# probably-nothing-labs/denormalized

Measured on AMD Instinct MI355X. Metric: rows/sec through window()+filter() on synthetic sensor stream, higher is better.
Workload: dtype f64

## Files before the change

### denormalized_amd/csrc/dz_internal.h

```cpp
#pragma once
#include <cstddef>
#include <cstdint>
#include <type_traits>
#include <hip/hip_runtime.h>

namespace dz {

constexpr int NB = 512;
constexpr int LOG_NB = 9;
constexpr int BLOCK = 256;
constexpr int WAVES_PER_BLOCK = BLOCK / 64;
constexpr int MAX_RANGES = 4096;
constexpr int ST_RECORDS = 2048;
constexpr int INTERN_STAGE_BYTES = 4096;

constexpr uint32_t META_KLOC_MASK = 0xFFFFu;
constexpr int META_WIDX_SHIFT = 16;
constexpr uint32_t META_WIDX_MASK = 0xFFFu;
constexpr int META_VALID_SHIFT = 28;

struct WinParams {
    int64_t s0;
    int64_t len_ms;
    int64_t slide_ms;
    int32_t nw;
    int32_t is_sliding;
};

struct FoldChunk {
    int32_t w_lo, w_hi;
    int32_t k_lo, k_hi;
    int64_t kcap;
    uint64_t row_base;
    int32_t bin_stride;
    int32_t tl_nw;
};

constexpr int MAX_EXTRA_COLS = 3;
struct FoldExtras {
    const double* vals[MAX_EXTRA_COLS] = {};
    const uint8_t* valid[MAX_EXTRA_COLS] = {};
    uint64_t* slab = nullptr;
    int64_t cells = 0;
    int32_t nx = 0;
};

void launch_gen(hipStream_t stream, uint64_t seed, int64_t t0, int64_t start_row,
                int64_t n, int64_t nkeys, int64_t rows_per_ms,
                int64_t* d_ts, int64_t* d_keys, int32_t* d_kid, double* d_vals);

void launch_intern(hipStream_t stream, const int32_t* d_offs, const char* d_data,
                   int64_t n,
                   uint4* tab ,
                   uint32_t* tab_row, uint32_t p_mask, uint32_t* id_off,
                   uint32_t* id_len, char* pool,
                   uint32_t* ctrs ,
                   uint32_t id_cap, uint32_t pool_cap, int32_t* out_kid,
                   uint32_t seq ,
                   uint64_t fp_mask ,
                   uint32_t* d_dbg);

void launch_intern_i64(hipStream_t stream, const int64_t* d_keys, int64_t n,
                       uint4* tab ,
                       uint32_t p_mask, int64_t* ikeys ,
                       uint32_t* ctrs ,
                       uint32_t id_cap, int32_t* out_kid,
                       uint32_t seq ,
                       uint64_t fp_mask ,
                       uint32_t* d_dbg);

void launch_gen_utf8(hipStream_t stream, uint64_t seed, int64_t start_row,
                     int64_t n, int64_t nkeys, int32_t* d_lens,
                     const int32_t* d_offs, char* d_data);

void launch_minmax(hipStream_t stream, const int64_t* d_ts, const int32_t* d_kid,
                   int64_t n, uint64_t* d_scalars);

void launch_hist(hipStream_t stream, const int32_t* d_kid, const int64_t* d_ts,
                 int64_t n, int64_t chunk, int C, const WinParams& wp,
                 uint32_t* d_ghist, uint64_t* d_scalars );

constexpr int SCAN_SSPLIT = 32;
void launch_scan(hipStream_t stream, const uint32_t* d_ghist, int C,
                 uint32_t* d_psum, uint32_t* d_bucket_base ,
                 uint32_t* d_gofs);

void launch_scatter(hipStream_t stream, const int32_t* d_kid, const int64_t* d_ts,
                    const double* d_vals, const uint8_t* d_validity ,
                    int64_t n, int64_t chunk, int C, int32_t st_rows,
                    const WinParams& wp, const uint32_t* d_gofs, uint4* d_grec,
                    uint32_t rec_limit, uint32_t* d_dbg );

constexpr int FOLD_GCAP = 256;

void launch_regroup_fold(hipStream_t stream, const uint4* d_grec,
                         const uint32_t* d_bucket_base,
                         const FoldChunk& fc, const int32_t* d_slot_of_widx,
                         uint64_t* s_cnt, double* s_min, double* s_max,
                         double* s_sum, uint64_t* s_first, int64_t slab_cells,
                         uint32_t* d_dbg, double* v_base, int64_t vslab_cells,
                         const FoldExtras& fx);

void launch_regroup_l1(hipStream_t stream, const uint4* d_grec,
                       const uint32_t* d_bucket_base,
                       const FoldChunk& fc, uint32_t* d_b1offs,
                       uint32_t* d_b1lens, uint4* d_grec2);

void launch_regroup_l2_fold(hipStream_t stream, const uint4* d_grec2,
                            const uint32_t* d_bucket_base,
                            const FoldChunk& fc, int nb1,
                            const uint32_t* d_b1offs, const uint32_t* d_b1lens,
                            const int32_t* d_slot_of_widx, uint64_t* s_cnt,
                            double* s_min, double* s_max, double* s_sum,
                            uint64_t* s_first, int64_t slab_cells,
                            uint32_t* d_dbg, double* v_base,
                            int64_t vslab_cells, const FoldExtras& fx);

struct EGatherSlots {
    int32_t s[16];
    uint64_t base[16];
};

struct EmitFilter {
    int32_t on;
    int32_t field;
    int32_t cmp;
    double lit;
};

__host__ __device__ inline bool emit_filter_pass(const EmitFilter& ef,
                                                 uint64_t cnt, double mn,
                                                 double mx, double sum) {
    double v;
// ... 50 lines not shown

void launch_emission_slabread(hipStream_t stream, const uint64_t* slab_first,
                              const uint64_t* slab_cnt, const double* slab_min,
                              const double* slab_max, const double* slab_sum,
                              uint64_t base, int64_t K, uint64_t* ekeys, uint32_t* ekid,
                              uint64_t* fkeys, uint32_t* fkid, uint32_t* fiota,
                              uint32_t* counter, uint32_t* counter2,
                              const EmitFilter& ef, uint64_t* ocnt, double* omin,
                              double* omax, double* osum, double* oavg,
                              uint8_t* oflags);
void launch_emission_sort(hipStream_t stream, int64_t K, uint64_t* fkeys,
                          uint64_t* skeys, uint32_t* fiota, uint32_t* okid,
                          uint32_t* counter2, uint32_t* rhist, uint32_t* roffs,
                          uint64_t max_key );
void launch_emission_group_read(hipStream_t stream, const uint64_t* s_base,
                                int64_t stride_u64, const EGatherSlots& slots,
                                int gcount, int64_t K, int64_t kcap,
                                const EmitFilter& ef, int cshift,
                                uint64_t* gkeys, uint32_t* gkid,
                                uint32_t* giota, uint64_t* gcnt_col,
                                double* gmin, double* gmax, double* gsum,
                                double* gavg, uint8_t* gflags, uint32_t* gtot,
                                uint32_t* gcnt);
void launch_emission_group_sort(hipStream_t stream, int64_t elem_cap,
                                int gcount, int cshift, uint64_t max_first,
                                uint64_t* gkeys, uint64_t* gskeys,
                                uint32_t* gkid, uint32_t* gokid,
                                uint32_t* giota, uint64_t* gcnt_col,
                                double* gmin, double* gmax, double* gsum,
                                double* gavg, uint8_t* gflags, uint32_t* gtot,
                                uint32_t* rhist, uint32_t* roffs, char* pout);

void launch_esort_small(hipStream_t stream, uint64_t* fkeys, uint64_t* skeys,
                        uint32_t* fiota, uint32_t* okid, uint32_t* counter2,
                        uint64_t max_key);
constexpr int EMIT_RCHUNK = 4096;
constexpr int EMIT_RBINS = 2048;

void launch_reset_slots(hipStream_t stream, const int32_t* d_slots, int ns,
                        int64_t kcap, uint64_t* s_cnt, uint64_t* s_first);

void launch_reset_slots_x(hipStream_t stream, const int32_t* d_slots, int ns,
                          int nx, int64_t kcap, uint64_t* x_slab);

void launch_egather_slabs(hipStream_t stream, const uint64_t* s_base,
                          int64_t stride_u64, EGatherSlots slots, int gcount,
                          uint64_t* out);
void launch_egather_slabs_var(hipStream_t stream, const uint64_t* s_base,
                              const double* v_base, int64_t kcap,
                              EGatherSlots slots, int gcount, uint64_t* out);
void launch_egather_slabs_x(hipStream_t stream, const uint64_t* s_base,
                            const uint64_t* x_slab, int nx, int64_t kcap,
                            EGatherSlots slots, int gcount, uint64_t* out);
void launch_arm_scalars(hipStream_t stream, uint64_t* scalars);

void launch_fill_i64(hipStream_t stream, int64_t* d_p, int64_t n, int64_t v);

struct JsonFields {
    char ts_name[32];
    char key_name[32];
    char val_name[32];
    int32_t ts_len, key_len, val_len;
};
void launch_json_count(hipStream_t stream, const char* d_buf, int64_t nbytes,
                       int C, int64_t chunk, int32_t tail_record,
                       uint32_t* d_cnt, uint32_t* d_base, uint32_t* d_tot);
void launch_json_parse(hipStream_t stream, const char* d_buf, int64_t nbytes,
                       int C, int64_t chunk, const JsonFields& jf,
                       const uint32_t* d_base, const uint32_t* d_tot,
                       int64_t* d_recoff, int64_t nrec, int64_t* o_ts,
                       int64_t* o_kbeg, int32_t* o_klen, double* o_val,
                       uint32_t* d_blocksum, uint32_t* d_ktot, int32_t* o_koff,
                       char* o_kdata, uint32_t* d_dbg);
void launch_gen_json(hipStream_t stream, uint64_t seed, int64_t t0,
                     int64_t start_row, int64_t n, int64_t nkeys,
                     int64_t rows_per_ms, int32_t* d_lens,
                     const int64_t* d_offs, char* d_data);

void launch_join_precheck(hipStream_t stream, const int64_t* d_trips,
                          const int64_t* d_drivers, int64_t n,
                          const int64_t* tab_trip, uint64_t p_mask,
                          uint32_t* d_pre);
void launch_join_build(hipStream_t stream, const int64_t* d_trips,
                       const int64_t* d_drivers, int64_t n, int64_t* tab_trip,
                       int64_t* tab_drv, uint64_t p_mask, uint32_t* d_dbg,
                       uint32_t* d_pre);
void launch_join_probe(hipStream_t stream, const int64_t* d_ts,
                       const int64_t* d_trips, const double* d_vals, int64_t n,
                       int64_t chunk, int C, const int64_t* tab_trip,
                       const int64_t* tab_drv, uint64_t p_mask,
                       int32_t* d_drvtmp, uint32_t* d_jcnt, uint32_t* d_mbase,
                       uint32_t* d_ubase, uint32_t* d_tot, int64_t* o_ts,
                       int32_t* o_kid, double* o_val, int64_t ubuf_base,
                       int64_t* u_ts, int64_t* u_trip, double* u_val);
void launch_zero_counters(hipStream_t stream, uint32_t* two_u32);
void launch_emission_permute(hipStream_t stream, int64_t K,
                             const uint32_t* counter2, const uint32_t* sidx,
                             const uint32_t* fkid, const uint64_t* ocnt,
                             const double* omin, const double* omax,
                             const double* osum, const double* oavg,
                             const uint8_t* oflags, char* out);

}
```

### denormalized_amd/csrc/kernels.hip

```cpp
#include "dz_internal.h"

#include <algorithm>

namespace dz {

__device__ __forceinline__ int64_t i64min(int64_t a, int64_t b) { return a < b ? a : b; }


__device__ __forceinline__ uint64_t splitmix64(uint64_t x) {
    x += 0x9e3779b97f4a7c15ULL;
    x = (x ^ (x >> 30)) * 0xbf58476d1ce4e5b9ULL;
    x = (x ^ (x >> 27)) * 0x94d049bb133111ebULL;
    return x ^ (x >> 31);
}

__device__ __forceinline__ int64_t snap_ms(int64_t ts, int64_t len_ms) {
    int64_t len_s = len_ms / 1000;
    if (len_s == 0) return ts - (ts % len_ms);
    return (ts / 1000) / len_s * len_s * 1000;
}

__device__ __forceinline__ int64_t floordiv(int64_t a, int64_t b) {
    int64_t q = a / b, r = a % b;
    return q - ((r != 0) & ((r < 0) != (b < 0)));
// ... 37 lines not shown
    if (blocks < 1) blocks = 1;
    hipLaunchKernelGGL(k_gen, dim3(blocks), dim3(BLOCK), 0, s, seed, t0,
                       start_row, n, nkeys, rows_per_ms, d_ts, d_keys, d_kid, d_vals);
}


__device__ __forceinline__ uint64_t fnv1a64(const char* p, int32_t len) {
    uint64_t h = 1469598103934665603ULL;
    for (int32_t i = 0; i < len; i++) {
        h ^= (uint8_t)p[i];
        h *= 1099511628211ULL;
    }
    return h;
}

__device__ __forceinline__ bool bytes_eq(const char* a, const char* b,
                                         int32_t len) {
    for (int32_t i = 0; i < len; i++)
        if (a[i] != b[i]) return false;
    return true;
}

constexpr uint32_t INTERN_INLINE_MAX = 16;

__device__ __forceinline__ uint64_t slot_fp(const uint4& v) {
    return (uint64_t)v.x | ((uint64_t)v.y << 32);
}

__device__ __forceinline__ uint64_t key_fp_bytes(const uint8_t* p, int32_t len,
                                                 uint64_t* klo, uint64_t* khi) {
    uint64_t lo = 0, hi = 0, fp = 1469598103934665603ULL;
    if ((uint32_t)len <= INTERN_INLINE_MAX) {
        const int32_t n0 = len < 8 ? len : 8;
        for (int32_t j = 0; j < n0; j++) {
            const uint64_t b = p[j];
            fp = (fp ^ b) * 1099511628211ULL;
            lo |= b << (8 * j);
        }
        for (int32_t j = 8; j < len; j++) {
            const uint64_t b = p[j];
            fp = (fp ^ b) * 1099511628211ULL;
            hi |= b << (8 * (j - 8));
        }
    } else {
        fp = fnv1a64((const char*)p, len);
    }
    *klo = lo;
    *khi = hi;
    return fp;
}

constexpr int INTERN_STAGE_GRAN = INTERN_STAGE_BYTES / 16 + 2;

__global__ __launch_bounds__(BLOCK) void k_intern_claim(const int32_t* offs,
        const char* data, int64_t n, uint4* tab, uint32_t* tab_row,
        const uint32_t* id_off, const uint32_t* id_len,
        const char* pool, uint32_t p_mask, uint64_t fp_mask, int32_t* out_kid,
        uint32_t* fresh_seq, uint32_t seq, uint32_t* dbg) {
    __shared__ int32_t s_offs[BLOCK + 1];
    __shared__ uint4 s_stage[INTERN_STAGE_GRAN];
    const int t = threadIdx.x;
    const int64_t ntiles = (n + BLOCK - 1) / BLOCK;
    for (int64_t tile = blockIdx.x; tile < ntiles; tile += gridDim.x) {
        const int64_t i0 = tile * BLOCK;
        const int rows = (int)i64min(BLOCK, n - i0);
        if (t < rows) s_offs[t] = offs[i0 + t];
        if (t == 0) s_offs[rows] = offs[i0 + rows];
        __syncthreads();
        const int32_t o_first = s_offs[0];
        const uint32_t span = (uint32_t)(s_offs[rows] - o_first);
        const bool staged = span <= (uint32_t)INTERN_STAGE_BYTES;
        uint32_t head = 0;
        if (staged) {
            if (span) {
                const char* a0 = data + o_first;
                head = (uint32_t)((uintptr_t)a0 & 15u);
                const uint4* g = (const uint4*)(a0 - head);
                const uint32_t ngran = (head + span + 15u) >> 4;
                for (uint32_t k = t; k < ngran; k += BLOCK) s_stage[k] = g[k];
            }
            __syncthreads();
        }
        const bool active = t < rows;
        const int64_t i = i0 + t;
        int32_t o0 = 0, len = 0;
        uint64_t klo = 0, khi = 0, fp = 0;
        if (active) {
            o0 = s_offs[t];
            len = s_offs[t + 1] - o0;
            if (staged) {
                const uint32_t q = head + (uint32_t)(o0 - o_first);
                fp = key_fp_bytes((const uint8_t*)s_stage + q, len, &klo,
                                  &khi);
            } else {
                fp = key_fp_bytes((const uint8_t*)data + o0, len, &klo, &khi);
            }
        }
        __syncthreads();
        if (!active) continue;
        const char* p = data + o0;
        fp &= fp_mask;
        if (!fp) fp = 1;
        uint32_t slot = (uint32_t)fp & p_mask;
        int32_t out;
        for (uint32_t probes = 0;; slot = (slot + 1) & p_mask) {
            const uint4 a = tab[(size_t)slot * 2];
            const uint4 b = tab[(size_t)slot * 2 + 1];
            const uint32_t cand = a.z;
            const uint32_t lo = a.w;
            const bool assigned = cand != ~0u;
            const bool fpeq = slot_fp(a) == fp;
            const uint64_t slo = (uint64_t)b.x | ((uint64_t)b.y << 32);
            const uint64_t shi = (uint64_t)b.z | ((uint64_t)b.w << 32);
            const bool inline_hit = assigned & fpeq &
                ((uint32_t)len <= INTERN_INLINE_MAX) &
                (lo == (((uint32_t)len << 6) | 63u)) & (slo == klo) &
                (shi == khi);
            if (inline_hit) {
                out = (int32_t)cand;
                break;
            }
            if (assigned) {
                const uint32_t clen = lo & 63u;
                const bool is_inline =
                    clen == 63u && (lo >> 6) <= INTERN_INLINE_MAX;
                if (fpeq && !is_inline) {
                    const bool fits = clen != 63u;
                    const uint32_t co = fits ? (lo >> 6) : id_off[cand];
                    const uint32_t cl = fits ? clen : id_len[cand];
                    if (cl == (uint32_t)len && bytes_eq(pool + co, p, len)) {
                        out = (int32_t)cand;
                        break;
                    }
                }
            } else {
                uint64_t got = __hip_atomic_load(
                    (const uint64_t*)tab + (size_t)slot * 4, __ATOMIC_RELAXED,
                    __HIP_MEMORY_SCOPE_AGENT);
                if (got == 0)
                    got = (uint64_t)atomicCAS(
                        (unsigned long long*)&tab[(size_t)slot * 2], 0ULL,
                        (unsigned long long)fp);
                if (got == 0 || got == fp) {
                    if (got == 0) tab_row[slot] = (uint32_t)i;
                    *fresh_seq = seq;
                    out = ~(int32_t)slot;
                    break;
                }
            }
            if (++probes > p_mask) {
                dbg[3] = 4;
                *fresh_seq = seq;
                out = ~(int32_t)slot;
                break;
            }
        }
        out_kid[i] = out;
    }
}

__global__ __launch_bounds__(BLOCK) void k_intern_assign(uint4* tab,
        uint32_t* tab_row, uint32_t p_count,
        const int32_t* offs, const char* data, uint32_t* id_off,
        uint32_t* id_len, char* pool, uint32_t* ctrs, uint32_t id_cap,
        uint32_t pool_cap, const uint32_t* fresh_seq, uint32_t seq,
        uint32_t* dbg) {
    if (*fresh_seq != seq) return;
    int64_t stride = (int64_t)gridDim.x * blockDim.x;
    for (int64_t sl = blockIdx.x * (int64_t)blockDim.x + threadIdx.x;
         sl < p_count; sl += stride) {
        uint4 v = tab[(size_t)sl * 2];
        if (slot_fp(v) == 0 || v.z != ~0u) continue;
        const uint32_t r = tab_row[sl];
        const int32_t o0 = offs[r];
        const int32_t len = offs[r + 1] - o0;
        const uint32_t nid = atomicAdd(&ctrs[0], 1u);
        const uint32_t po = atomicAdd(&ctrs[1], (uint32_t)len);
        if (nid >= id_cap || po + (uint32_t)len > pool_cap) {
            dbg[3] = nid >= id_cap ? 1 : 2;
            continue;
        }
        uint64_t klo = 0, khi = 0;
        for (int32_t j = 0; j < len; j++) {
            const uint8_t c = (uint8_t)data[o0 + j];
            pool[po + j] = (char)c;
            if (j < 8) klo |= (uint64_t)c << (8 * j);
            else if (j < (int32_t)INTERN_INLINE_MAX)
                khi |= (uint64_t)c << (8 * (j - 8));
        }
        id_off[nid] = po;
        id_len[nid] = (uint32_t)len;
        v.z = nid;
        if ((uint32_t)len <= INTERN_INLINE_MAX) {
            v.w = ((uint32_t)len << 6) | 63u;
            tab[(size_t)sl * 2 + 1] = make_uint4((uint32_t)klo,
                (uint32_t)(klo >> 32), (uint32_t)khi, (uint32_t)(khi >> 32));
        } else {
            v.w = (len <= 62 && po < (1u << 26)) ? ((po << 6) | (uint32_t)len)
                                                 : 0xFFFFFFFFu;
        }
        tab[(size_t)sl * 2] = v;
    }
}

__global__ __launch_bounds__(BLOCK) void k_intern_lookup(const int32_t* offs,
        const char* data, int64_t n, const uint4* tab,
        const uint32_t* id_off, const uint32_t* id_len, const char* pool,
        int32_t* out_kid, const uint32_t* fresh_seq, uint32_t seq,
        uint32_t* dbg) {
    if (*fresh_seq != seq) return;
    int64_t stride = (int64_t)gridDim.x * blockDim.x;
    for (int64_t i = blockIdx.x * (int64_t)blockDim.x + threadIdx.x; i < n;
         i += stride) {
        const int32_t v = out_kid[i];
        if (v >= 0) continue;
        const uint32_t slot = (uint32_t)~v;
        const uint32_t cand = tab[(size_t)slot * 2].z;
        int32_t id = 0;
        if (cand == ~0u) {
            dbg[3] = 5;
        } else {
            const int32_t o0 = offs[i];
            const int32_t len = offs[i + 1] - o0;
            const bool eq = id_len[cand] == (uint32_t)len &&
                            bytes_eq(pool + id_off[cand], data + o0, len);
            if (eq) id = (int32_t)cand;
            else dbg[3] = 6;
        }
        out_kid[i] = id;
    }
}

void launch_intern(hipStream_t s, const int32_t* d_offs, const char* d_data,
                   int64_t n, uint4* tab, uint32_t* tab_row, uint32_t p_mask,
                   uint32_t* id_off, uint32_t* id_len, char* pool,
                   uint32_t* ctrs, uint32_t id_cap, uint32_t pool_cap,
                   int32_t* out_kid, uint32_t seq, uint64_t fp_mask,
                   uint32_t* dbg) {
    int blocks = (int)std::min<int64_t>((n + BLOCK - 1) / BLOCK, 2048);
    if (blocks < 1) blocks = 1;
    const uint32_t P = p_mask + 1;
    int sblocks = (int)std::min<uint32_t>((P + BLOCK - 1) / BLOCK, 2048);
    uint32_t* fresh_seq = ctrs + 2;
    hipLaunchKernelGGL(k_intern_claim, dim3(blocks), dim3(BLOCK), 0, s, d_offs,
                       d_data, n, tab, tab_row, id_off, id_len,
                       pool, p_mask, fp_mask, out_kid, fresh_seq, seq, dbg);
    hipLaunchKernelGGL(k_intern_assign, dim3(sblocks), dim3(BLOCK), 0, s,
                       tab, tab_row, P, d_offs, d_data, id_off,
                       id_len, pool, ctrs, id_cap, pool_cap, fresh_seq, seq,
                       dbg);
    hipLaunchKernelGGL(k_intern_lookup, dim3(blocks), dim3(BLOCK), 0, s,
                       d_offs, d_data, n, tab, id_off,
                       id_len, pool, out_kid, fresh_seq, seq, dbg);
}


constexpr uint64_t I64_ZERO_CLAIM = 1;

__global__ __launch_bounds__(BLOCK) void k_intern_i64_claim(
        const int64_t* keys, int64_t n, uint4* tab, uint32_t p_mask,
        uint64_t fp_mask, int32_t* out_kid, uint32_t* fresh_seq, uint32_t seq,
        uint32_t* dbg) {
    const int64_t stride = (int64_t)gridDim.x * blockDim.x;
    for (int64_t i = blockIdx.x * (int64_t)blockDim.x + threadIdx.x; i < n;
         i += stride) {
        const uint64_t key = (uint64_t)keys[i];
        const bool zero = key == 0;
        const uint64_t want = zero ? I64_ZERO_CLAIM : key;
        uint32_t slot = zero ? p_mask + 1
                             : (uint32_t)(splitmix64(key) & fp_mask) & p_mask;
        int32_t out;
        for (uint32_t probes = 0;; slot = (slot + 1) & p_mask) {
            const uint4 a = tab[slot];
            if (a.z != ~0u) {
                if (slot_fp(a) == want) {
                    out = (int32_t)a.z;
                    break;
                }
            } else {
                uint64_t got = __hip_atomic_load(
                    (const uint64_t*)tab + (size_t)slot * 2, __ATOMIC_RELAXED,
                    __HIP_MEMORY_SCOPE_AGENT);
                if (got == 0)
                    got = (uint64_t)atomicCAS((unsigned long long*)&tab[slot],
                                              0ULL, (unsigned long long)want);
                if (got == 0 || got == want) {
                    if (got == 0) ((uint32_t*)&tab[slot])[3] = (uint32_t)i;
                    *fresh_seq = seq;
                    out = ~(int32_t)slot;
                    break;
                }
            }
            if (++probes > p_mask) {
                dbg[3] = 4;
                *fresh_seq = seq;
                out = ~(int32_t)slot;
                break;
            }
        }
// ... 56 lines not shown
                       n, tab, out_kid, fresh_seq, seq, dbg);
}

__device__ __forceinline__ int32_t dec_digits(uint64_t k) {
    int32_t d = 1;
    while (k >= 10) { k /= 10; d++; }
    return d;
}

__global__ void k_gen_keylens(uint64_t seed, int64_t start_row, int64_t n,
                              int64_t nkeys, int32_t* lens) {
    int64_t stride = (int64_t)gridDim.x * blockDim.x;
    for (int64_t i = blockIdx.x * (int64_t)blockDim.x + threadIdx.x; i < n;
         i += stride) {
        uint64_t r = splitmix64(seed ^ (0x9e3779b97f4a7c15ULL *
                                        (uint64_t)(start_row + i + 1)));
        lens[i] = 7 + dec_digits(r % (uint64_t)nkeys);
    }
}

__global__ void k_gen_keyfill(uint64_t seed, int64_t start_row, int64_t n,
                              int64_t nkeys, const int32_t* offs, char* data) {
    const char* pfx = "sensor_";
    int64_t stride = (int64_t)gridDim.x * blockDim.x;
    for (int64_t i = blockIdx.x * (int64_t)blockDim.x + threadIdx.x; i < n;
         i += stride) {
        uint64_t r = splitmix64(seed ^ (0x9e3779b97f4a7c15ULL *
                                        (uint64_t)(start_row + i + 1)));
        uint64_t k = r % (uint64_t)nkeys;
        char* p = data + offs[i];
        for (int j = 0; j < 7; j++) p[j] = pfx[j];
        int32_t len = offs[i + 1] - offs[i];
        for (int32_t j = len - 1; j >= 7; j--) {
            p[j] = (char)('0' + (k % 10));
            k /= 10;
        }
    }
}

void launch_gen_utf8(hipStream_t s, uint64_t seed, int64_t start_row, int64_t n,
                     int64_t nkeys, int32_t* d_lens, const int32_t* d_offs,
                     char* d_data) {
    int blocks = (int)std::min<int64_t>((n + BLOCK - 1) / BLOCK, 2048);
    if (blocks < 1) blocks = 1;
    if (d_lens)
        hipLaunchKernelGGL(k_gen_keylens, dim3(blocks), dim3(BLOCK), 0, s, seed,
                           start_row, n, nkeys, d_lens);
    if (d_data)
        hipLaunchKernelGGL(k_gen_keyfill, dim3(blocks), dim3(BLOCK), 0, s, seed,
                           start_row, n, nkeys, d_offs, d_data);
}


__device__ __forceinline__ uint64_t map_i64(int64_t x) {
    return (uint64_t)x ^ 0x8000000000000000ULL;
}

__global__ __launch_bounds__(BLOCK) void k_minmax(const int64_t* ts,
        const int32_t* kid, int64_t n, uint64_t* scalars) {
    __shared__ uint64_t red[3][WAVES_PER_BLOCK];
    uint64_t mn = ~0ULL, mx = 0, km = 0;
    int64_t stride = (int64_t)gridDim.x * blockDim.x;
    for (int64_t i = blockIdx.x * (int64_t)blockDim.x + threadIdx.x; i < n; i += stride) {
        uint64_t t = map_i64(ts[i]);
        mn = min(mn, t);
        mx = max(mx, t);
        if (kid) km = max(km, (uint64_t)(uint32_t)kid[i]);
    }
    for (int o = 32; o > 0; o >>= 1) {
        mn = min(mn, (uint64_t)__shfl_down((unsigned long long)mn, o));
        mx = max(mx, (uint64_t)__shfl_down((unsigned long long)mx, o));
        km = max(km, (uint64_t)__shfl_down((unsigned long long)km, o));
    }
    const int wave = threadIdx.x >> 6;
    if ((threadIdx.x & 63) == 0) {
        red[0][wave] = mn;
        red[1][wave] = mx;
        red[2][wave] = km;
    }
    __syncthreads();
    if (threadIdx.x == 0) {
        for (int w = 1; w < WAVES_PER_BLOCK; w++) {
            mn = min(mn, red[0][w]);
            mx = max(mx, red[1][w]);
            km = max(km, red[2][w]);
        }
        atomicMin((unsigned long long*)&scalars[0], (unsigned long long)mn);
        atomicMax((unsigned long long*)&scalars[1], (unsigned long long)mx);
        atomicMax((unsigned long long*)&scalars[2], (unsigned long long)km);
    }
}

void launch_minmax(hipStream_t s, const int64_t* d_ts, const int32_t* d_kid,
                   int64_t n, uint64_t* d_scalars) {
    int blocks = (int)std::min<int64_t>((n + BLOCK - 1) / BLOCK, 512);
    if (blocks < 1) blocks = 1;
    hipLaunchKernelGGL(k_minmax, dim3(blocks), dim3(BLOCK), 0, s, d_ts, d_kid, n,
                       d_scalars);
}


__global__ __launch_bounds__(BLOCK) void k_hist(const int32_t* kid,
        const int64_t* ts, int64_t n, int64_t chunk, WinParams wp,
        uint32_t* ghist, uint64_t* scalars) {
    __shared__ uint32_t h[NB];
    __shared__ uint64_t red[3][WAVES_PER_BLOCK];
    for (int t = threadIdx.x; t < NB; t += BLOCK) h[t] = 0;
    __syncthreads();
    int64_t lo = blockIdx.x * chunk;
    int64_t hi = i64min(n, lo + chunk);
    uint64_t mn = ~0ULL, mx = 0, km = 0;
    for (int64_t i = lo + threadIdx.x; i < hi; i += BLOCK) {
        uint32_t k = (uint32_t)kid[i];
        uint32_t m = 1;
        if (wp.is_sliding) {
            int32_t jm, mm;
            row_windows(ts[i], wp, &jm, &mm);
            m = (uint32_t)mm;
        }
        if (scalars) {
            uint64_t t = map_i64(ts[i]);
            mn = min(mn, t);
            mx = max(mx, t);
            km = max(km, (uint64_t)k);
        }
        if (m) atomicAdd(&h[k & (NB - 1)], m);
    }
    __syncthreads();
    for (int t = threadIdx.x; t < NB; t += BLOCK)
        ghist[(int64_t)blockIdx.x * NB + t] = h[t];
    if (scalars) {
        for (int o = 32; o > 0; o >>= 1) {
            mn = min(mn, (uint64_t)__shfl_down((unsigned long long)mn, o));
            mx = max(mx, (uint64_t)__shfl_down((unsigned long long)mx, o));
            km = max(km, (uint64_t)__shfl_down((unsigned long long)km, o));
        }
        const int wave = threadIdx.x >> 6;
        if ((threadIdx.x & 63) == 0) {
            red[0][wave] = mn;
            red[1][wave] = mx;
            red[2][wave] = km;
        }
        __syncthreads();
        if (threadIdx.x == 0) {
            for (int w = 1; w < WAVES_PER_BLOCK; w++) {
                mn = min(mn, red[0][w]);
                mx = max(mx, red[1][w]);
                km = max(km, red[2][w]);
            }
            atomicMin((unsigned long long*)&scalars[0], (unsigned long long)mn);
            atomicMax((unsigned long long*)&scalars[1], (unsigned long long)mx);
            atomicMax((unsigned long long*)&scalars[2], (unsigned long long)km);
        }
    }
}

void launch_hist(hipStream_t s, const int32_t* d_kid, const int64_t* d_ts,
                 int64_t n, int64_t chunk, int C, const WinParams& wp,
                 uint32_t* d_ghist, uint64_t* d_scalars) {
    hipLaunchKernelGGL(k_hist, dim3(C), dim3(BLOCK), 0, s, d_kid, d_ts, n, chunk,
                       wp, d_ghist, d_scalars);
}


constexpr int SSPLIT = SCAN_SSPLIT;

__global__ void k_scan_partial(const uint32_t* ghist, int C, int cs,
                               uint32_t* psum) {
    int bkt = blockIdx.x * blockDim.x + threadIdx.x;
    int seg = blockIdx.y;
    if (bkt >= NB) return;
    int c0 = seg * cs, c1 = min(C, c0 + cs);
    uint32_t s = 0;
    for (int c = c0; c < c1; c++) s += ghist[(int64_t)c * NB + bkt];
    psum[(int64_t)seg * NB + bkt] = s;
}

__global__ __launch_bounds__(NB) void k_scan_base(const uint32_t* psum,
                                                  uint32_t* base) {
    __shared__ uint32_t part[NB];
    const int bkt = threadIdx.x;
    uint32_t t = 0;
    for (int g = 0; g < SSPLIT; g++) t += psum[(int64_t)g * NB + bkt];
    part[bkt] = t;
    __syncthreads();
    for (int o = 1; o < NB; o <<= 1) {
        uint32_t v = (bkt >= o) ? part[bkt - o] : 0;
        __syncthreads();
        part[bkt] += v;
        __syncthreads();
    }
    base[bkt] = bkt ? part[bkt - 1] : 0;
    if (bkt == NB - 1) base[NB] = part[NB - 1];
}

__global__ void k_scan_offsets(const uint32_t* ghist, int C, int cs,
                               const uint32_t* psum, const uint32_t* base,
                               uint32_t* gofs) {
    int bkt = blockIdx.x * blockDim.x + threadIdx.x;
    int seg = blockIdx.y;
    if (bkt >= NB) return;
    uint32_t run = base[bkt];
    for (int g = 0; g < seg; g++) run += psum[(int64_t)g * NB + bkt];
    int c0 = seg * cs, c1 = min(C, c0 + cs);
    for (int c = c0; c < c1; c++) {
        uint32_t t = ghist[(int64_t)c * NB + bkt];
        gofs[(int64_t)c * NB + bkt] = run;
        run += t;
    }
}

void launch_scan(hipStream_t s, const uint32_t* d_ghist, int C,
                 uint32_t* d_psum, uint32_t* d_base, uint32_t* d_gofs) {
    int cs = (C + SSPLIT - 1) / SSPLIT;
// ... 1127 lines not shown
}

__global__ void k_egather_slabs_var(const uint64_t* __restrict__ s_base,
                                    const uint64_t* __restrict__ v_base,
                                    int64_t kcap, dz::EGatherSlots slots,
                                    uint64_t* __restrict__ out) {
    const int g = blockIdx.y;
    const int64_t slot = slots.s[g];
    const uint64_t* src = s_base + slot * (5 * kcap);
    const uint64_t* m2 = v_base + slot * (2 * kcap) + kcap;
    uint64_t* dst = out + (int64_t)g * (6 * kcap);
    for (int64_t i = (int64_t)blockIdx.x * blockDim.x + threadIdx.x;
         i < 6 * kcap; i += (int64_t)gridDim.x * blockDim.x)
        dst[i] = i < 5 * kcap ? src[i] : m2[i - 5 * kcap];
}

void dz::launch_egather_slabs_var(hipStream_t s, const uint64_t* s_base,
                                  const double* v_base, int64_t kcap,
                                  dz::EGatherSlots slots, int gcount,
                                  uint64_t* out) {
    int bx = (int)std::min<int64_t>((6 * kcap + dz::BLOCK - 1) / dz::BLOCK,
                                    512);
    dim3 grid(bx, gcount);
    hipLaunchKernelGGL(k_egather_slabs_var, grid, dim3(dz::BLOCK), 0, s,
                       s_base, (const uint64_t*)v_base, kcap, slots, out);
}

__global__ void k_egather_slabs_x(const uint64_t* __restrict__ s_base,
                                  const uint64_t* __restrict__ x_slab, int nx,
                                  int64_t kcap, dz::EGatherSlots slots,
                                  uint64_t* __restrict__ out) {
    const int g = blockIdx.y;
    const int64_t slot = slots.s[g];
    const int64_t ncell = (int64_t)(5 + 4 * nx) * kcap;
    const uint64_t* src = s_base + slot * (5 * kcap);
    const uint64_t* xs = x_slab + slot * ((int64_t)(4 * nx) * kcap);
    uint64_t* dst = out + (int64_t)g * ncell;
    for (int64_t i = (int64_t)blockIdx.x * blockDim.x + threadIdx.x;
         i < ncell; i += (int64_t)gridDim.x * blockDim.x)
        dst[i] = i < 5 * kcap ? src[i] : xs[i - 5 * kcap];
}

void dz::launch_egather_slabs_x(hipStream_t s, const uint64_t* s_base,
                                const uint64_t* x_slab, int nx, int64_t kcap,
                                dz::EGatherSlots slots, int gcount,
                                uint64_t* out) {
    int bx = (int)std::min<int64_t>(
        ((int64_t)(5 + 4 * nx) * kcap + dz::BLOCK - 1) / dz::BLOCK, 512);
    dim3 grid(bx, gcount);
    hipLaunchKernelGGL(k_egather_slabs_x, grid, dim3(dz::BLOCK), 0, s, s_base,
                       x_slab, nx, kcap, slots, out);
}

__global__ void k_arm_scalars(uint64_t* __restrict__ s) {
    s[0] = ~0ULL;
    s[1] = 0ULL;
    s[2] = 0ULL;
}

void dz::launch_arm_scalars(hipStream_t st, uint64_t* s) {
    hipLaunchKernelGGL(k_arm_scalars, dim3(1), dim3(1), 0, st, s);
}

__global__ void k_zero2(uint32_t* __restrict__ p) {
    p[0] = 0;
    p[1] = 0;
}

void dz::launch_zero_counters(hipStream_t st, uint32_t* p) {
    hipLaunchKernelGGL(k_zero2, dim3(1), dim3(1), 0, st, p);
}

__global__ void k_epermute(const uint32_t* __restrict__ counter2,
                           const uint32_t* __restrict__ sidx,
                           const uint32_t* __restrict__ fkid,
                           const uint64_t* __restrict__ ocnt,
                           const double* __restrict__ omin,
                           const double* __restrict__ omax,
                           const double* __restrict__ osum,
                           const double* __restrict__ oavg,
                           const uint8_t* __restrict__ oflags,
                           char* __restrict__ out) {
    const uint32_t nt = *counter2;
    const auto o = dz::packed_cols(out, nt);
    int64_t stride = (int64_t)gridDim.x * blockDim.x;
    for (int64_t i = blockIdx.x * (int64_t)blockDim.x + threadIdx.x; i < nt;
         i += stride) {
        const uint32_t j = sidx[i];
        const uint32_t k = fkid[j];
        o.key[i] = (int64_t)k;
        o.cnt[i] = ocnt[j];
        o.min[i] = omin[j];
        o.max[i] = omax[j];
        o.sum[i] = osum[j];
        o.avg[i] = oavg[j];
        o.kid[i] = k;
        o.flags[i] = oflags[j] & 1;
    }
}

void dz::launch_emission_permute(hipStream_t st, int64_t K,
                                 const uint32_t* counter2, const uint32_t* sidx,
                                 const uint32_t* fkid, const uint64_t* ocnt,
                                 const double* omin, const double* omax,
                                 const double* osum, const double* oavg,
                                 const uint8_t* oflags, char* out) {
    int blocks = (int)std::min<int64_t>((K + dz::BLOCK - 1) / dz::BLOCK, 2048);
    if (blocks < 1) blocks = 1;
    hipLaunchKernelGGL(k_epermute, dim3(blocks), dim3(dz::BLOCK), 0, st,
                       counter2, sidx, fkid, ocnt, omin, omax, osum, oavg,
                       oflags, out);
}


// ... 861 lines not shown
```

### denormalized_amd/csrc/window_op.cpp

```cpp
#include "dz_internal.h"
#include "denormalized_amd.h"

#include <algorithm>
#include <cmath>
#include <cstdio>
#include <cstring>
#include <deque>
#include <map>
#include <string>
#include <unordered_map>
#include <atomic>
#include <condition_variable>
#include <memory>
#include <mutex>
#include <thread>
#include <vector>

namespace {

std::string g_err;

int64_t snap_ms_host(int64_t ts, int64_t len_ms) {
    int64_t len_s = len_ms / 1000;
    if (len_s == 0) return ts - (ts % len_ms);
// ... 1589 lines not shown
        int g1c = (int)(std::min(closed.size(), g0 + gstep) - g0);
        dz_status st;
        if (grouped_ok) {
            st = enqueue_group_device(op, cl, g1c);
        } else if (!dev_path_g && op->e_gbufs[0]) {
            st = enqueue_group_host(op, cl, g1c);
        } else if (op->host_route()) {
            op->err = "internal: variance / multi-column aggregates need the "
                      "pinned group buffers (allocation missing)";
            st = DZ_ERR;
        } else {
            st = enqueue_per_close(op, cl, g1c, &g1c);
        }
        if (st != DZ_OK) return DZ_ERR;
        g0 += (size_t)g1c;
    }
    return DZ_OK;
}


static void quiesce(dz_window_op* op) {
    hipStreamSynchronize(op->stream);
    if (op->i_stream) hipStreamSynchronize(op->i_stream);
}

static dz_status ensure_scratch(dz_window_op* op, int C, int64_t nrec) {
    if (C > op->C_cap) {
        quiesce(op);
        for (int i = 0; i < 2; i++) {
            hipFree(op->d_ghist[i]); hipFree(op->d_gofs[i]);
            CHK(op, hipMalloc(&op->d_ghist[i], (size_t)C * dz::NB * 4));
            CHK(op, hipMalloc(&op->d_gofs[i], (size_t)C * dz::NB * 4));
            if (!op->d_total[i]) {
                CHK(op, hipMalloc(&op->d_total[i],
                                  (size_t)dz::SCAN_SSPLIT * dz::NB * 4));
                CHK(op, hipMalloc(&op->d_base[i], (dz::NB + 1) * 4));
            }
        }
        op->C_cap = C;
    }
    if (nrec > op->rec_cap) {
        quiesce(op);
        hipFree(op->d_grec);
        CHK(op, hipMalloc(&op->d_grec, (size_t)nrec * 16));
        op->rec_cap = nrec;
    }
    return DZ_OK;
}

static dz_status stage_core(dz_window_op* op, int64_t n, const int64_t* d_ts,
                            const int32_t* d_kid, const double* d_vals,
                            const uint8_t* d_valbm, bool keys_are_dense,
                            bool deferred, bool borrow = false,
                            const dz_window_op::XCols* xc = nullptr) {
    if (n >= (1LL << 31)) {
        op->err = "batch exceeds 2^31 rows; push smaller batches";
        return DZ_ERR;
    }
    const bool sliding = op->slide_ms > 0;
    int C = (int)std::min<int64_t>(512, std::max<int64_t>(1, (n + 8191) / 8192));
    int64_t chunk = (n + C - 1) / C;
    int b = op->next_buf;
    op->next_buf ^= 1;
    hipStream_t s = deferred ? op->i_stream : op->stream;
    if (deferred && !borrow) {
        HostTimer ht(op, "h_stage");
        if (n > op->s_in_cap[b]) {
            quiesce(op);
            hipFree(op->d_sts[b]); hipFree(op->d_skid[b]); hipFree(op->d_svals[b]);
            CHK(op, hipMalloc(&op->d_sts[b], (size_t)n * 8));
            CHK(op, hipMalloc(&op->d_skid[b], (size_t)n * 4));
            CHK(op, hipMalloc(&op->d_svals[b], (size_t)n * 8));
            op->s_in_cap[b] = n;
        }
        if (op->consumed_valid[b])
            CHK(op, hipStreamWaitEvent(s, op->ev_consumed[b], 0));
        CHK(op, hipMemcpyAsync(op->d_sts[b], d_ts, (size_t)n * 8,
                               hipMemcpyDeviceToDevice, s));
        CHK(op, hipMemcpyAsync(op->d_skid[b], d_kid, (size_t)n * 4,
                               hipMemcpyDeviceToDevice, s));
        CHK(op, hipMemcpyAsync(op->d_svals[b], d_vals, (size_t)n * 8,
                               hipMemcpyDeviceToDevice, s));
        CHK(op, hipEventRecord(op->ev_staged[b], s));
        d_ts = op->d_sts[b];
        d_kid = op->d_skid[b];
        d_vals = op->d_svals[b];
    } else if (deferred && op->consumed_valid[b]) {
        CHK(op, hipStreamWaitEvent(s, op->ev_consumed[b], 0));
    } else if (op->consumed_valid[b]) {
        CHK(op, hipStreamWaitEvent(s, op->ev_consumed[b], 0));
    }
    dz::launch_arm_scalars(s, op->d_scalars[b]);
    dz::WinParams wp;
    memset(&wp, 0, sizeof(wp));
    wp.len_ms = op->len_ms;
    wp.slide_ms = op->slide_ms;
    wp.is_sliding = sliding;
    if (!sliding) {
        if (ensure_scratch(op, C, n) != DZ_OK) return DZ_ERR;
        timed_on(op, s, "hist", (double)n * 12, [&] {
            dz::launch_hist(s, d_kid, d_ts, n, chunk, C, wp,
                            op->d_ghist[b], op->d_scalars[b]);
        });
        timed_on(op, s, "scan", (double)C * dz::NB * 12, [&] {
            dz::launch_scan(s, op->d_ghist[b], C, op->d_total[b],
                            op->d_base[b], op->d_gofs[b]);
        });
    } else {
        timed_on(op, s, "minmax", (double)n * 12, [&] {
            dz::launch_minmax(s, d_ts, keys_are_dense ? d_kid : nullptr,
                              n, op->d_scalars[b]);
        });
    }
    CHK(op, hipMemcpyAsync(op->h_scalars + 3 * b, op->d_scalars[b], 24,
                           hipMemcpyDeviceToHost, s));
    CHK(op, hipEventRecord(op->ev_ready[b], s));
    op->pend.active = true;
    op->pend.sliding = sliding;
    op->pend.dense = keys_are_dense;
    op->pend.deferred = deferred;
    op->pend.buf = b;
    op->pend.C = C;
    op->pend.n = n;
    op->pend.chunk = chunk;
    op->pend.ts = d_ts;
    op->pend.kid = d_kid;
    op->pend.vals = d_vals;
    op->pend.valbm = d_valbm;
    op->pend.x = xc ? *xc : dz_window_op::XCols();
    if (deferred && !borrow) {
        HostTimer ht(op, "h_stage");
        event_spin(op->ev_staged[b]);
    }
    return DZ_OK;
}

static dz_status process_batch(dz_window_op* op, const dz_window_op::Pend& P);

static dz_status process_pending(dz_window_op* op) {
    if (!op->pend.active) return DZ_OK;
    CHK(op, hipSetDevice(op->device));
    dz_window_op::Pend P = op->pend;
    op->pend.active = false;
    return process_batch(op, P);
}

static dz_status process_batch(dz_window_op* op, const dz_window_op::Pend& P) {
    const bool sliding = P.sliding;
    const bool keys_are_dense = P.dense;
    const int64_t n = P.n, chunk = P.chunk;
    const int C = P.C;
    const int b = P.buf;
    const int64_t* d_ts = P.ts;
    const int32_t* d_kid = P.kid;
    const double* d_vals = P.vals;
// ... 455 lines not shown
    return DZ_OK;
}

extern "C" dz_status dz_debug_intern_fp_bits(dz_window_op* op, int32_t bits) {
    if (!op) return DZ_ERR;
    if (op->d_itab) {
        op->err = "dz_debug_intern_fp_bits is legal only before the first "
                  "device utf8 push";
        return DZ_ERR;
    }
    if (op->d_i64tab) {
        op->err = "dz_debug_intern_fp_bits is legal only before the first "
                  "device i64 push";
        return DZ_ERR;
    }
    if (bits < 1 || bits > 64) {
        op->err = "dz_debug_intern_fp_bits: bits must be in 1..64";
        return DZ_ERR;
    }
    op->i_fpmask = bits == 64 ? ~0ULL : ((1ULL << bits) - 1);
    return DZ_OK;
}

extern "C" dz_status dz_window_op_push_device_utf8(dz_window_op* op,
        int64_t n_rows, const int64_t* d_ts_ms, const int32_t* d_key_offsets,
        const char* d_key_data, const double* d_vals) {
    if (!op) return DZ_ERR;
    if (op->key_kind != DZ_KEY_UTF8 || op->no_group) {
        op->err = "push_device_utf8 requires key_kind DZ_KEY_UTF8";
        return DZ_ERR;
    }
    if (!op->dict_utf8.empty()) {
        op->err = "cannot mix host utf8 pushes and device utf8 pushes on one "
                  "operator (two dictionaries would assign conflicting ids)";
        return DZ_ERR;
    }
    dz_window_op::XCols xc;
    if (take_extras(op, n_rows, &xc) != DZ_OK) return DZ_ERR;
    CHK(op, hipSetDevice(op->device));
    if (n_rows <= 0) return process_pending(op);
    int C = (int)std::min<int64_t>(512,
                                   std::max<int64_t>(1, (n_rows + 8191) / 8192));
    if (op->pend.active &&
        (C > op->C_cap || (op->slide_ms == 0 && n_rows > op->rec_cap))) {
        if (process_pending(op) != DZ_OK) return DZ_ERR;
    }
    if (ensure_intern(op, n_rows) != DZ_OK) return DZ_ERR;
    dz_window_op::Pend prev = op->pend;
    op->pend.active = false;
    int b = op->next_buf;
    if (op->consumed_valid[b])
        CHK(op, hipStreamWaitEvent(op->i_stream, op->ev_consumed[b], 0));
    if (++op->i_seq == 0) op->i_seq = 1;
    timed_on(op, op->i_stream, "intern", (double)n_rows * 18, [&] {
        dz::launch_intern(op->i_stream, d_key_offsets, d_key_data, n_rows,
                          op->d_itab, op->d_itab_row,
                          op->i_pmask, op->d_ioff, op->d_ilen, op->d_ipool,
                          op->d_ictrs, op->i_idcap, op->i_poolcap,
                          op->d_ikid[b], op->i_seq, op->i_fpmask, op->d_dbg);
    });
    if (stage_core(op, n_rows, d_ts_ms, op->d_ikid[b], d_vals, nullptr,
                   true, true,
                   true, &xc) != DZ_OK)
        return DZ_ERR;
    if (prev.active) return process_batch(op, prev);
    return DZ_OK;
}

extern "C" dz_status dz_window_op_push_device_i64(dz_window_op* op,
        int64_t n_rows, const int64_t* d_ts_ms, const int64_t* d_keys,
        const double* d_vals) {
    if (!op) return DZ_ERR;
    if (op->key_kind != DZ_KEY_INT64 || op->no_group) {
        op->err = "push_device_i64 requires key_kind DZ_KEY_INT64";
        return DZ_ERR;
    }
    if (!op->dict_i64.empty()) {
        op->err = "cannot mix host int64 pushes and device i64 pushes on one "
                  "operator (two dictionaries would assign conflicting ids)";
        return DZ_ERR;
    }
    if ((uintptr_t)d_keys & 7) {
        op->err = "push_device_i64: d_keys must be 8-byte aligned";
        return DZ_ERR;
    }
    dz_window_op::XCols xc;
    if (take_extras(op, n_rows, &xc) != DZ_OK) return DZ_ERR;
    CHK(op, hipSetDevice(op->device));
    if (n_rows <= 0) return process_pending(op);
    int C = (int)std::min<int64_t>(512,
                                   std::max<int64_t>(1, (n_rows + 8191) / 8192));
    if (op->pend.active &&
        (C > op->C_cap || (op->slide_ms == 0 && n_rows > op->rec_cap))) {
        if (process_pending(op) != DZ_OK) return DZ_ERR;
    }
    if (ensure_intern_i64(op, n_rows) != DZ_OK) return DZ_ERR;
    dz_window_op::Pend prev = op->pend;
    op->pend.active = false;
    int b = op->next_buf;
    if (op->consumed_valid[b])
        CHK(op, hipStreamWaitEvent(op->i_stream, op->ev_consumed[b], 0));
    if (++op->i_seq == 0) op->i_seq = 1;
    timed_on(op, op->i_stream, "intern_i64", (double)n_rows * 12, [&] {
        dz::launch_intern_i64(op->i_stream, d_keys, n_rows, op->d_i64tab,
                              op->i_pmask, op->d_ikeys, op->d_ictrs,
                              op->i_idcap, op->d_ikid[b], op->i_seq,
                              op->i_fpmask, op->d_dbg);
    });
    if (stage_core(op, n_rows, d_ts_ms, op->d_ikid[b], d_vals, nullptr,
                   true, true,
                   true, &xc) != DZ_OK)
        return DZ_ERR;
    if (prev.active) return process_batch(op, prev);
    return DZ_OK;
}

// ... 910 lines not shown
```

Measured before the change: 16.39 billion.

## Fuse per-chunk histogram and min/max into intern claim kernel for tumbling windows

For tumbling windows on string keys, the intern claim kernel now also builds the per-chunk key histogram and reduces timestamp min/max and max key id. It launches C×CLAIM_SPLIT blocks aligned to chunks, and the ghist buffer is zeroed in the arm-scalars kernel. The separate hist kernel becomes gated on a device-side fresh-sequence flag, so it only reruns when new keys were assigned, which is when the claim pass left some rows unresolved. This removes a full pass over kid/ts in the common steady-state case. The cost is a restructured claim grid with possible lower parallelism, plus global atomics on the histogram when the split is greater than one.

```diff
diff --git a/denormalized_amd/csrc/dz_internal.h b/denormalized_amd/csrc/dz_internal.h
--- a/denormalized_amd/csrc/dz_internal.h
+++ b/denormalized_amd/csrc/dz_internal.h
@@ -48,6 +48,18 @@
 void launch_gen(hipStream_t stream, uint64_t seed, int64_t t0, int64_t start_row,
                 int64_t n, int64_t nkeys, int64_t rows_per_ms,
                 int64_t* d_ts, int64_t* d_keys, int32_t* d_kid, double* d_vals);
+
+#ifndef DZ_CLAIM_SPLIT
+#define DZ_CLAIM_SPLIT 4
+#endif
+constexpr int CLAIM_SPLIT = DZ_CLAIM_SPLIT;
+struct ClaimHist {
+    const int64_t* d_ts;
+    int64_t chunk;
+    int C;
+    uint32_t* d_ghist;
+    uint64_t* d_scalars;
+};
 
 void launch_intern(hipStream_t stream, const int32_t* d_offs, const char* d_data,
                    int64_t n,
@@ -58,7 +70,8 @@
                    uint32_t id_cap, uint32_t pool_cap, int32_t* out_kid,
                    uint32_t seq ,
                    uint64_t fp_mask ,
-                   uint32_t* d_dbg);
+                   uint32_t* d_dbg,
+                   const ClaimHist* ch );
 
 void launch_intern_i64(hipStream_t stream, const int64_t* d_keys, int64_t n,
                        uint4* tab ,
@@ -79,6 +92,12 @@
 void launch_hist(hipStream_t stream, const int32_t* d_kid, const int64_t* d_ts,
                  int64_t n, int64_t chunk, int C, const WinParams& wp,
                  uint32_t* d_ghist, uint64_t* d_scalars );
+
+void launch_hist_gated(hipStream_t stream, const int32_t* d_kid,
+                       const int64_t* d_ts, int64_t n, int64_t chunk, int C,
+                       const WinParams& wp, uint32_t* d_ghist,
+                       uint64_t* d_scalars, const uint32_t* fresh_seq,
+                       uint32_t seq);
 
 constexpr int SCAN_SSPLIT = 32;
 void launch_scan(hipStream_t stream, const uint32_t* d_ghist, int C,
@@ -235,7 +254,8 @@
 void launch_egather_slabs_x(hipStream_t stream, const uint64_t* s_base,
                             const uint64_t* x_slab, int nx, int64_t kcap,
                             EGatherSlots slots, int gcount, uint64_t* out);
-void launch_arm_scalars(hipStream_t stream, uint64_t* scalars);
+void launch_arm_scalars(hipStream_t stream, uint64_t* scalars,
+                        uint32_t* zero = nullptr, int64_t nzero = 0);
 
 void launch_fill_i64(hipStream_t stream, int64_t* d_p, int64_t n, int64_t v);
 
diff --git a/denormalized_amd/csrc/kernels.hip b/denormalized_amd/csrc/kernels.hip
--- a/denormalized_amd/csrc/kernels.hip
+++ b/denormalized_amd/csrc/kernels.hip
@@ -113,18 +113,41 @@
 
 constexpr int INTERN_STAGE_GRAN = INTERN_STAGE_BYTES / 16 + 2;
 
+__device__ __forceinline__ uint64_t map_i64(int64_t x) {
+    return (uint64_t)x ^ 0x8000000000000000ULL;
+}
+
+template <bool HIST>
 __global__ __launch_bounds__(BLOCK) void k_intern_claim(const int32_t* offs,
         const char* data, int64_t n, uint4* tab, uint32_t* tab_row,
         const uint32_t* id_off, const uint32_t* id_len,
         const char* pool, uint32_t p_mask, uint64_t fp_mask, int32_t* out_kid,
-        uint32_t* fresh_seq, uint32_t seq, uint32_t* dbg) {
+        uint32_t* fresh_seq, uint32_t seq, uint32_t* dbg, const int64_t* ts,
+        int64_t chunk, int split, uint32_t* ghist, uint64_t* scalars) {
     __shared__ int32_t s_offs[BLOCK + 1];
     __shared__ uint4 s_stage[INTERN_STAGE_GRAN];
+    __shared__ uint32_t h[HIST ? NB : 1];
+    __shared__ uint64_t red[3][WAVES_PER_BLOCK];
     const int t = threadIdx.x;
-    const int64_t ntiles = (n + BLOCK - 1) / BLOCK;
-    for (int64_t tile = blockIdx.x; tile < ntiles; tile += gridDim.x) {
-        const int64_t i0 = tile * BLOCK;
-        const int rows = (int)i64min(BLOCK, n - i0);
+    int64_t base = 0, end = n, tile_b = blockIdx.x, tile_step = gridDim.x;
+    int64_t tile_e = (n + BLOCK - 1) / BLOCK;
+    const int c = HIST ? (int)(blockIdx.x / (uint32_t)split) : 0;
+    if (HIST) {
+        for (int k = t; k < NB; k += BLOCK) h[k] = 0;
+        base = c * chunk;
+        end = i64min(n, base + chunk);
+        const int64_t nt = end > base ? (end - base + BLOCK - 1) / BLOCK : 0;
+        const int64_t per = (nt + split - 1) / split;
+        tile_b = (int64_t)(blockIdx.x % (uint32_t)split) * per;
+        tile_e = i64min(nt, tile_b + per);
+        tile_step = 1;
+    }
+    uint64_t mn = ~0ULL, mx = 0, km = 0;
+    for (int64_t tile = tile_b; tile < tile_e; tile += tile_step) {
+        const int64_t i0 = base + tile * BLOCK;
+        const int rows = (int)i64min(BLOCK, end - i0);
+        int64_t tsv = 0;
+        if (HIST && t < rows) tsv = ts[i0 + t];
         if (t < rows) s_offs[t] = offs[i0 + t];
         if (t == 0) s_offs[rows] = offs[i0 + rows];
         __syncthreads();
@@ -217,6 +240,45 @@
             }
         }
         out_kid[i] = out;
+        if (HIST && out >= 0) {
+            atomicAdd(&h[(uint32_t)out & (NB - 1)], 1u);
+            const uint64_t tm = map_i64(tsv);
+            mn = min(mn, tm);
+            mx = max(mx, tm);
+            km = max(km, (uint64_t)(uint32_t)out);
+        }
+    }
+    if (!HIST) return;
+    __syncthreads();
+    uint32_t* gh = ghist + (int64_t)c * NB;
+    for (int k = t; k < NB; k += BLOCK) {
+        const uint32_t v = h[k];
+        if (split == 1) gh[k] = v;
+        else if (v) atomicAdd(&gh[k], v);
+    }
+    for (int o = 32; o > 0; o >>= 1) {
+        mn = min(mn, (uint64_t)__shfl_down((unsigned long long)mn, o));
+        mx = max(mx, (uint64_t)__shfl_down((unsigned long long)mx, o));
+        km = max(km, (uint64_t)__shfl_down((unsigned long long)km, o));
+    }
+    const int wave = t >> 6;
+    if ((t & 63) == 0) {
+        red[0][wave] = mn;
+        red[1][wave] = mx;
+        red[2][wave] = km;
+    }
+    __syncthreads();
+    if (t == 0) {
+        for (int w = 1; w < WAVES_PER_BLOCK; w++) {
+            mn = min(mn, red[0][w]);
+            mx = max(mx, red[1][w]);
+            km = max(km, red[2][w]);
+        }
+        if (mn <= mx) {
+            atomicMin((unsigned long long*)&scalars[0], (unsigned long long)mn);
+            atomicMax((unsigned long long*)&scalars[1], (unsigned long long)mx);
+            atomicMax((unsigned long long*)&scalars[2], (unsigned long long)km);
+        }
     }
 }
 
@@ -297,15 +359,23 @@
                    uint32_t* id_off, uint32_t* id_len, char* pool,
                    uint32_t* ctrs, uint32_t id_cap, uint32_t pool_cap,
                    int32_t* out_kid, uint32_t seq, uint64_t fp_mask,
-                   uint32_t* dbg) {
+                   uint32_t* dbg, const ClaimHist* ch) {
     int blocks = (int)std::min<int64_t>((n + BLOCK - 1) / BLOCK, 2048);
     if (blocks < 1) blocks = 1;
     const uint32_t P = p_mask + 1;
     int sblocks = (int)std::min<uint32_t>((P + BLOCK - 1) / BLOCK, 2048);
     uint32_t* fresh_seq = ctrs + 2;
-    hipLaunchKernelGGL(k_intern_claim, dim3(blocks), dim3(BLOCK), 0, s, d_offs,
-                       d_data, n, tab, tab_row, id_off, id_len,
-                       pool, p_mask, fp_mask, out_kid, fresh_seq, seq, dbg);
+    if (ch)
+        hipLaunchKernelGGL(k_intern_claim<true>, dim3(ch->C * CLAIM_SPLIT),
+                           dim3(BLOCK), 0, s, d_offs, d_data, n, tab, tab_row,
+                           id_off, id_len, pool, p_mask, fp_mask, out_kid,
+                           fresh_seq, seq, dbg, ch->d_ts, ch->chunk,
+                           CLAIM_SPLIT, ch->d_ghist, ch->d_scalars);
+    else
+        hipLaunchKernelGGL(k_intern_claim<false>, dim3(blocks), dim3(BLOCK), 0,
+                           s, d_offs, d_data, n, tab, tab_row, id_off, id_len,
+                           pool, p_mask, fp_mask, out_kid, fresh_seq, seq, dbg,
+                           nullptr, 0, 1, nullptr, nullptr);
     hipLaunchKernelGGL(k_intern_assign, dim3(sblocks), dim3(BLOCK), 0, s,
                        tab, tab_row, P, d_offs, d_data, id_off,
                        id_len, pool, ctrs, id_cap, pool_cap, fresh_seq, seq,
@@ -468,10 +538,6 @@
 }
 
 
-__device__ __forceinline__ uint64_t map_i64(int64_t x) {
-    return (uint64_t)x ^ 0x8000000000000000ULL;
-}
-
 __global__ __launch_bounds__(BLOCK) void k_minmax(const int64_t* ts,
         const int32_t* kid, int64_t n, uint64_t* scalars) {
     __shared__ uint64_t red[3][WAVES_PER_BLOCK];
@@ -516,8 +582,8 @@
 }
 
 
-__global__ __launch_bounds__(BLOCK) void k_hist(const int32_t* kid,
-        const int64_t* ts, int64_t n, int64_t chunk, WinParams wp,
+__device__ __forceinline__ void hist_pass(const int32_t* kid,
+        const int64_t* ts, int64_t n, int64_t chunk, const WinParams& wp,
         uint32_t* ghist, uint64_t* scalars) {
     __shared__ uint32_t h[NB];
     __shared__ uint64_t red[3][WAVES_PER_BLOCK];
@@ -571,11 +637,33 @@
     }
 }
 
+__global__ __launch_bounds__(BLOCK) void k_hist(const int32_t* kid,
+        const int64_t* ts, int64_t n, int64_t chunk, WinParams wp,
+        uint32_t* ghist, uint64_t* scalars) {
+    hist_pass(kid, ts, n, chunk, wp, ghist, scalars);
+}
+
+__global__ __launch_bounds__(BLOCK) void k_hist_gated(const int32_t* kid,
+        const int64_t* ts, int64_t n, int64_t chunk, WinParams wp,
+        uint32_t* ghist, uint64_t* scalars, const uint32_t* fresh_seq,
+        uint32_t seq) {
+    if (*fresh_seq != seq) return;
+    hist_pass(kid, ts, n, chunk, wp, ghist, scalars);
+}
+
 void launch_hist(hipStream_t s, const int32_t* d_kid, const int64_t* d_ts,
                  int64_t n, int64_t chunk, int C, const WinParams& wp,
                  uint32_t* d_ghist, uint64_t* d_scalars) {
     hipLaunchKernelGGL(k_hist, dim3(C), dim3(BLOCK), 0, s, d_kid, d_ts, n, chunk,
                        wp, d_ghist, d_scalars);
+}
+
+void launch_hist_gated(hipStream_t s, const int32_t* d_kid, const int64_t* d_ts,
+                       int64_t n, int64_t chunk, int C, const WinParams& wp,
+                       uint32_t* d_ghist, uint64_t* d_scalars,
+                       const uint32_t* fresh_seq, uint32_t seq) {
+    hipLaunchKernelGGL(k_hist_gated, dim3(C), dim3(BLOCK), 0, s, d_kid, d_ts, n,
+                       chunk, wp, d_ghist, d_scalars, fresh_seq, seq);
 }
 
 
@@ -1809,14 +1897,26 @@
                        x_slab, nx, kcap, slots, out);
 }
 
-__global__ void k_arm_scalars(uint64_t* __restrict__ s) {
-    s[0] = ~0ULL;
-    s[1] = 0ULL;
-    s[2] = 0ULL;
-}
-
-void dz::launch_arm_scalars(hipStream_t st, uint64_t* s) {
-    hipLaunchKernelGGL(k_arm_scalars, dim3(1), dim3(1), 0, st, s);
+__global__ void k_arm_scalars(uint64_t* __restrict__ s, uint4* __restrict__ z,
+                              int nz16) {
+    const int i = blockIdx.x * blockDim.x + threadIdx.x;
+    if (i == 0) {
+        s[0] = ~0ULL;
+        s[1] = 0ULL;
+        s[2] = 0ULL;
+    }
+    if (i < nz16) z[i] = make_uint4(0, 0, 0, 0);
+}
+
+void dz::launch_arm_scalars(hipStream_t st, uint64_t* s, uint32_t* zero,
+                            int64_t nzero) {
+    const int nz16 = zero ? (int)(nzero / 4) : 0;
+    if (nz16 > 0)
+        hipLaunchKernelGGL(k_arm_scalars, dim3((nz16 + dz::BLOCK - 1) / dz::BLOCK),
+                           dim3(dz::BLOCK), 0, st, s, (uint4*)zero, nz16);
+    else
+        hipLaunchKernelGGL(k_arm_scalars, dim3(1), dim3(1), 0, st, s,
+                           (uint4*)nullptr, 0);
 }
 
 __global__ void k_zero2(uint32_t* __restrict__ p) {
diff --git a/denormalized_amd/csrc/window_op.cpp b/denormalized_amd/csrc/window_op.cpp
--- a/denormalized_amd/csrc/window_op.cpp
+++ b/denormalized_amd/csrc/window_op.cpp
@@ -1665,7 +1665,8 @@
                             const int32_t* d_kid, const double* d_vals,
                             const uint8_t* d_valbm, bool keys_are_dense,
                             bool deferred, bool borrow = false,
-                            const dz_window_op::XCols* xc = nullptr) {
+                            const dz_window_op::XCols* xc = nullptr,
+                            bool claim_hist = false) {
     if (n >= (1LL << 31)) {
         op->err = "batch exceeds 2^31 rows; push smaller batches";
         return DZ_ERR;
@@ -1703,7 +1704,7 @@
     } else if (op->consumed_valid[b]) {
         CHK(op, hipStreamWaitEvent(s, op->ev_consumed[b], 0));
     }
-    dz::launch_arm_scalars(s, op->d_scalars[b]);
+    if (!claim_hist) dz::launch_arm_scalars(s, op->d_scalars[b]);
     dz::WinParams wp;
     memset(&wp, 0, sizeof(wp));
     wp.len_ms = op->len_ms;
@@ -1711,9 +1712,14 @@
     wp.is_sliding = sliding;
     if (!sliding) {
         if (ensure_scratch(op, C, n) != DZ_OK) return DZ_ERR;
-        timed_on(op, s, "hist", (double)n * 12, [&] {
-            dz::launch_hist(s, d_kid, d_ts, n, chunk, C, wp,
-                            op->d_ghist[b], op->d_scalars[b]);
+        timed_on(op, s, "hist", claim_hist ? 0.0 : (double)n * 12, [&] {
+            if (claim_hist)
+                dz::launch_hist_gated(s, d_kid, d_ts, n, chunk, C, wp,
+                                      op->d_ghist[b], op->d_scalars[b],
+                                      op->d_ictrs + 2, op->i_seq);
+            else
+                dz::launch_hist(s, d_kid, d_ts, n, chunk, C, wp,
+                                op->d_ghist[b], op->d_scalars[b]);
         });
         timed_on(op, s, "scan", (double)C * dz::NB * 12, [&] {
             dz::launch_scan(s, op->d_ghist[b], C, op->d_total[b],
@@ -2275,16 +2281,32 @@
     if (op->consumed_valid[b])
         CHK(op, hipStreamWaitEvent(op->i_stream, op->ev_consumed[b], 0));
     if (++op->i_seq == 0) op->i_seq = 1;
-    timed_on(op, op->i_stream, "intern", (double)n_rows * 18, [&] {
+    const bool claim_hist = op->slide_ms == 0;
+    dz::ClaimHist ch = {};
+    if (claim_hist) {
+        if (ensure_scratch(op, C, n_rows) != DZ_OK) return DZ_ERR;
+        ch.d_ts = d_ts_ms;
+        ch.C = C;
+        ch.chunk = (n_rows + C - 1) / C;
+        ch.d_ghist = op->d_ghist[b];
+        ch.d_scalars = op->d_scalars[b];
+        const bool zero = dz::CLAIM_SPLIT > 1;
+        dz::launch_arm_scalars(op->i_stream, op->d_scalars[b],
+                               zero ? op->d_ghist[b] : nullptr,
+                               (int64_t)C * dz::NB);
+    }
+    timed_on(op, op->i_stream, "intern",
+             (double)n_rows * (claim_hist ? 26 : 18), [&] {
         dz::launch_intern(op->i_stream, d_key_offsets, d_key_data, n_rows,
                           op->d_itab, op->d_itab_row,
                           op->i_pmask, op->d_ioff, op->d_ilen, op->d_ipool,
                           op->d_ictrs, op->i_idcap, op->i_poolcap,
-                          op->d_ikid[b], op->i_seq, op->i_fpmask, op->d_dbg);
+                          op->d_ikid[b], op->i_seq, op->i_fpmask, op->d_dbg,
+                          claim_hist ? &ch : nullptr);
     });
     if (stage_core(op, n_rows, d_ts_ms, op->d_ikid[b], d_vals, nullptr,
                    true, true,
-                   true, &xc) != DZ_OK)
+                   true, &xc, claim_hist) != DZ_OK)
         return DZ_ERR;
     if (prev.active) return process_batch(op, prev);
     return DZ_OK;
```

Measured after the change: 16.40 billion, median of 2. No clear change (+0.1%).
